# Snoworday/instance-segmentation-attention

Measured on NVIDIA B200. Metric: images/sec (pred.py inference, train step at 1/2/4/8 B200) vs host-CPU ref, higher is better.
Workload: dtype f32 (hot path fp32-accurate: bf16x3 tensor-core products, fp32 accumulation; cuDNN backbone convolutions at PyTorch's default TF32)

## Files before the change

### instance-segmentation-attention_b200/csrc/proj_gemm.cu

```cuda
#include "isa_common.cuh"
#include "isa_tcgen05.cuh"

namespace {

constexpr int kBM = 256;
constexpr int kBNMax = 256;
constexpr int kBK = 32;
constexpr int kStages = 3;
constexpr int kProducerThreads = 512;
constexpr int kThreadsTotal = kProducerThreads;
constexpr int kTileA = kBM * kBK * 2;
constexpr int kTileB = kBNMax * kBK * 2;
constexpr int kStageBytes = 2 * kTileA + 2 * kTileB;
constexpr int kGroupStride = (kBK / 8) * 128;
constexpr int kMaxSeg = 4;

struct Seg {
  const float* ptr;
  long long ld;
  long long shift;
  int cols;
  int v0;
  int pos_div, pos_mod, pos_step;
  int ones;
};

struct Operand {
  Seg seg[kMaxSeg];
  int nseg;
  int mn_major;
  int extent;
};

struct GemmParams {
  Operand a, b;
  long long K;
  long long k_per_split;
  float* out;
  long long ldc;
  long long out_rows;
  int out_cols;
  int bn;
  const unsigned char* b_packed;
  int n_iter_total;
};

struct Chunk {
  const float* p;
  long long step;
  int off;
  int k0;
  int tail;
  int seg;
};

__device__ __forceinline__ void plan_chunk(const Operand& op, long long mn_base, int groups, long long k_lo, int q, Chunk& c) {
  c.p = nullptr; c.step = 0; c.off = 0; c.k0 = 0; c.tail = 8; c.seg = -1;
  if (op.mn_major) {
    const int k8 = q & 7, mgl = (q >> 3) & 3, rest = q >> 5, kg = rest & 3, mg = (rest >> 2) * 4 + mgl;
    if (mg >= groups) { c.off = -1; return; }
    c.off = mg * kGroupStride + kg * 128 + k8 * 16;
    c.k0 = (int)k_lo + kg * 8 + k8;
    const int mn0 = (int)mn_base + mg * 8;
    if (mn0 >= op.extent) return;
    int si = 0;
#pragma unroll
    for (int j = 1; j < kMaxSeg; ++j)
      if (j < op.nseg && mn0 >= op.seg[j].v0) si = j;
    const Seg& sg = op.seg[si];
    const int col = mn0 - sg.v0;
    if (col >= sg.cols) return;
    c.tail = sg.cols - col < 8 ? sg.cols - col : 8;
    c.seg = (sg.ones || sg.pos_step != 0) ? si : -1;
    c.step = (long long)kBK * sg.ld;
    c.p = sg.ones ? reinterpret_cast<const float*>(&op)  : sg.ptr + ((long long)c.k0 + sg.shift) * sg.ld + col;
  } else {
    const int r8 = q & 7, kc = (q >> 3) & 3, rg = q >> 5;
    if (rg >= groups) { c.off = -1; return; }
    c.off = rg * kGroupStride + kc * 128 + r8 * 16;
    c.k0 = (int)k_lo + kc * 8;
    const long long mn = mn_base + rg * 8 + r8;
    if (mn >= op.extent) return;
    c.step = kBK;
    c.p = op.seg[0].ptr + mn * op.seg[0].ld + c.k0;
  }
}

__device__ __forceinline__ void load_chunk(const Operand& op, const Chunk& c, int it, int k_hi, float (&v)[8]) {
#pragma unroll
  for (int i = 0; i < 8; ++i) v[i] = 0.f;
  if (c.p == nullptr) return;
  const int k = c.k0 + it * kBK;
  if (k >= k_hi) return;
  const float* p = c.p + (long long)it * c.step;
  if (op.mn_major) {
    if (c.seg >= 0) {
      const Seg& sg = op.seg[c.seg];
      if (sg.ones) {
#pragma unroll
        for (int i = 0; i < 8; ++i) v[i] = i < c.tail ? 1.f : 0.f;
        return;
      }
      const int pos = (int)(((unsigned)k / (unsigned)sg.pos_div) % (unsigned)sg.pos_mod) + sg.pos_step;
      if (pos < 0 || pos >= sg.pos_mod) return;
    }
    if (c.tail == 8) {
      const float4 a = __ldg(reinterpret_cast<const float4*>(p));
      const float4 b = __ldg(reinterpret_cast<const float4*>(p + 4));
      v[0] = a.x; v[1] = a.y; v[2] = a.z; v[3] = a.w; v[4] = b.x; v[5] = b.y; v[6] = b.z; v[7] = b.w;
    } else {
#pragma unroll
      for (int i = 0; i < 8; ++i)
        if (i < c.tail) v[i] = __ldg(p + i);
    }
  } else {
    if (k + 8 <= k_hi) {
      const float4 a = __ldg(reinterpret_cast<const float4*>(p));
      const float4 b = __ldg(reinterpret_cast<const float4*>(p + 4));
      v[0] = a.x; v[1] = a.y; v[2] = a.z; v[3] = a.w; v[4] = b.x; v[5] = b.y; v[6] = b.z; v[7] = b.w;
    } else {
#pragma unroll
      for (int i = 0; i < 8; ++i)
        if (k + i < k_hi) v[i] = __ldg(p + i);
    }
  }
}

__device__ __forceinline__ void store_split8(unsigned char* hi_tile, unsigned char* lo_tile, int off, const float (&v)[8]) {
  uint4 h, l;
  split2(v[0], v[1], h.x, l.x);
  split2(v[2], v[3], h.y, l.y);
  split2(v[4], v[5], h.z, l.z);
  split2(v[6], v[7], h.w, l.w);
  *reinterpret_cast<uint4*>(hi_tile + off) = h;
  *reinterpret_cast<uint4*>(lo_tile + off) = l;
}

__global__ void __launch_bounds__(kProducerThreads) pack_operand_kernel(const __grid_constant__ Operand op, int bn, int k_total, unsigned char* __restrict__ dst) {
  const int it = blockIdx.x, nt = blockIdx.y;
  const int n0 = nt * bn;
  int width = op.extent - n0;
  width = width > bn ? bn : ((width + 15) & ~15);
  unsigned char* hi = dst + ((size_t)nt * gridDim.x + it) * 2 * (size_t)bn * (kBK * 2);
  unsigned char* lo = hi + (size_t)bn * (kBK * 2);
#pragma unroll 1
  for (int i = 0; i < kBNMax * (kBK / 8) / kProducerThreads; ++i) {
    Chunk c;
    plan_chunk(op, n0, width / 8, 0, threadIdx.x + i * kProducerThreads, c);
    if (c.off < 0) continue;
    float v[8];
    load_chunk(op, c, it, k_total, v);
    store_split8(hi, lo, c.off, v);
  }
}

template <bool PACKED_B>
__global__ void __launch_bounds__(kThreadsTotal, 1) proj_gemm_kernel(const __grid_constant__ GemmParams p) {
  extern __shared__ __align__(16) unsigned char smem_raw_g[];
  unsigned char* sm = smem_raw_g + ((128u - (smem_u32(smem_raw_g) & 127u)) & 127u);
  __shared__ uint64_t s_full[kStages], s_empty[kStages], s_done;
  __shared__ uint32_t s_tmem;
  const int tid = threadIdx.x;
  const int warp = __shfl_sync(0xffffffffu, tid >> 5, 0);
  const long long m0 = (long long)blockIdx.y * kBM;
  const int n0 = blockIdx.x * p.bn;
  const long long k_lo = (long long)blockIdx.z * p.k_per_split;
  const int k_hi = (int)((k_lo + p.k_per_split < p.K) ? k_lo + p.k_per_split : p.K);
  const int n_iter = (int)((k_hi - k_lo + kBK - 1) / kBK);
  int bn = p.b.extent - n0;
  bn = bn > p.bn ? p.bn : ((bn + 15) & ~15);
  const int n_acc = (p.a.extent - m0 > 128) ? 2 : 1;

  if (tid == 0) {
    for (int s = 0; s < kStages; ++s) { mbar_init(&s_full[s], kProducerThreads / 32 + (PACKED_B ? 1 : 0)); mbar_init(&s_empty[s], 1); }
    mbar_init(&s_done, 1);
    fence_barrier_init();
  }
  if (warp == 0) tmem_alloc(&s_tmem, 512);
  tc_fence_before();
  __syncthreads();
  tc_fence_after();
  const uint32_t tmem = s_tmem;

  {
    const uint32_t el = elect_one();
    const uint32_t idesc = make_idesc(128, bn) | ((uint32_t)(p.a.mn_major ? 1 : 0) << 15) | ((uint32_t)(p.b.mn_major ? 1 : 0) << 16);
    constexpr int NA = kBM * (kBK / 8) / kProducerThreads;
    constexpr int NB = PACKED_B ? 1 : kBNMax * (kBK / 8) / kProducerThreads;
    Chunk ca[NA], cb[NB];
    float va[NA][8], vb[NB][8], na[NA][8], nb_[NB][8];
#pragma unroll
    for (int i = 0; i < NA; ++i) {
      plan_chunk(p.a, m0, n_acc * 16, k_lo, tid + i * kProducerThreads, ca[i]);
      if (ca[i].off >= 0) load_chunk(p.a, ca[i], 0, k_hi, va[i]);
    }
    if (!PACKED_B) {
#pragma unroll
      for (int i = 0; i < NB; ++i) {
        plan_chunk(p.b, n0, bn / 8, k_lo, tid + i * kProducerThreads, cb[i]);
        if (cb[i].off >= 0) load_chunk(p.b, cb[i], 0, k_hi, vb[i]);
      }
    }
    const size_t pk_tile = (size_t)p.bn * (kBK * 2);
    const int lane_p = tid & 31;
    auto k_block = [&](int it, float (&cur_a)[NA][8], float (&cur_b)[NB][8], float (&nxt_a)[NA][8], float (&nxt_b)[NB][8]) {
      const int s = it % kStages;
      const uint32_t ph = (uint32_t)(it / kStages) & 1u;
      if (it + 1 < n_iter) {
#pragma unroll
        for (int i = 0; i < NA; ++i)
          if (ca[i].off >= 0) load_chunk(p.a, ca[i], it + 1, k_hi, nxt_a[i]);
        if (!PACKED_B) {
#pragma unroll
          for (int i = 0; i < NB; ++i)
            if (cb[i].off >= 0) load_chunk(p.b, cb[i], it + 1, k_hi, nxt_b[i]);
        }
      }
      if (lane_p == 0) mbar_wait(&s_empty[s], ph ^ 1u);
      __syncwarp();
      unsigned char* st = sm + s * kStageBytes;
      if (PACKED_B && tid == 0) {
        const unsigned char* src = p.b_packed + ((size_t)blockIdx.x * p.n_iter_total + (size_t)(k_lo / kBK) + it) * 2 * pk_tile;
        const uint32_t bytes = (uint32_t)bn * (kBK * 2);
        mbar_arrive_expect_tx(&s_full[s], 2 * bytes);
        tma_bulk_g2s(st + 2 * kTileA, src, bytes, &s_full[s]);
        tma_bulk_g2s(st + 2 * kTileA + kTileB, src + pk_tile, bytes, &s_full[s]);
      }
#pragma unroll
      for (int i = 0; i < NA; ++i)
        if (ca[i].off >= 0) store_split8(st, st + kTileA, ca[i].off, cur_a[i]);
      if (!PACKED_B) {
#pragma unroll
        for (int i = 0; i < NB; ++i)
          if (cb[i].off >= 0) store_split8(st + 2 * kTileA, st + 2 * kTileA + kTileB, cb[i].off, cur_b[i]);
      }
      fence_proxy_async();
      __syncwarp();
      if (lane_p == 0) mbar_arrive(&s_full[s]);
      if (warp == 0) {
        mbar_wait(&s_full[s], ph);
        tc_fence_after();
        const uint32_t base = smem_u32(st);
        const uint64_t b_hi = make_desc(base + 2 * kTileA, 128, kGroupStride), b_lo = make_desc(base + 2 * kTileA + kTileB, 128, kGroupStride);
        for (int acc = 0; acc < n_acc; ++acc) {
          const uint32_t a_off = (uint32_t)acc * (16 * kGroupStride);
          const uint64_t a_hi = make_desc(base + a_off, 128, kGroupStride), a_lo = make_desc(base + kTileA + a_off, 128, kGroupStride);
          const uint32_t d = tmem + (uint32_t)acc * 256u;
#pragma unroll
          for (int kk = 0; kk < kBK / 16; ++kk) {
            const uint64_t ko = (uint64_t)((kk * 256) >> 4);
            umma_bf16_e(el, d, a_hi + ko, b_hi + ko, idesc, (it > 0 || kk > 0) ? 1u : 0u);
            umma_bf16_e(el, d, a_hi + ko, b_lo + ko, idesc, 1u);
            umma_bf16_e(el, d, a_lo + ko, b_hi + ko, idesc, 1u);
          }
        }
        umma_commit_e(el, &s_empty[s]);
        if (it + 1 == n_iter) umma_commit_e(el, &s_done);
      }
    };
    for (int it = 0; it < n_iter; it += 2) {
      k_block(it, va, vb, na, nb_);
      if (it + 1 < n_iter) k_block(it + 1, na, nb_, va, vb);
    }
    if (warp < 4 * n_acc) {
      mbar_wait(&s_done, 0);
      tc_fence_after();
      const int lane = tid & 31;
      const int acc = warp >> 2, quarter = warp & 3;
      const uint32_t t_row = tmem + ((uint32_t)(quarter * 32) << 16) + (uint32_t)acc * 256u;
      float* stg = reinterpret_cast<float*>(sm) + warp * (32 * 36);
      const long long row_base = m0 + acc * 128 + quarter * 32;
      float* obase = p.out + ((long long)blockIdx.z * p.out_rows + row_base) * p.ldc + n0;
      for (int c0 = 0; c0 < bn; c0 += 32) {
        uint32_t d[32];
        if (bn - c0 >= 32) {
          tmem_ld32_issue(t_row + c0, d);
          tmem_ld32_wait(d);
        } else {
          uint32_t e[16];
          tmem_ld16_issue(t_row + c0, e);
          tmem_ld16_wait(e);
#pragma unroll
          for (int i = 0; i < 16; ++i) { d[i] = e[i]; d[i + 16] = 0u; }
        }
#pragma unroll
        for (int i = 0; i < 32; i += 4) *reinterpret_cast<uint4*>(stg + lane * 36 + i) = make_uint4(d[i], d[i + 1], d[i + 2], d[i + 3]);
        __syncwarp();
        int lim = p.out_cols - (n0 + c0);
        if (lim > bn - c0) lim = bn - c0;
        const int col = (lane & 7) * 4;
#pragma unroll
        for (int j = 0; j < 8; ++j) {
          const int r = j * 4 + (lane >> 3);
          const uint4 v = *reinterpret_cast<const uint4*>(stg + r * 36 + col);
          if (row_base + r < p.out_rows) {
            float* o = obase + (long long)r * p.ldc + c0 + col;
            if (col + 4 <= lim) *reinterpret_cast<uint4*>(o) = v;
            else {
              if (col + 0 < lim) o[0] = __uint_as_float(v.x);
              if (col + 1 < lim) o[1] = __uint_as_float(v.y);
              if (col + 2 < lim) o[2] = __uint_as_float(v.z);
              if (col + 3 < lim) o[3] = __uint_as_float(v.w);
            }
          }
        }
        __syncwarp();
      }
      tc_fence_before();
    }
  }
  __syncthreads();
  if (warp == 0) {
    tc_fence_after();
    tmem_dealloc(tmem, 512);
  }
}

__global__ void __launch_bounds__(256) renet_wgrad_reduce_kernel(const float* __restrict__ part, int splits, long long rows_pad, long long ldc,
                                                                 int n, int cin, int cb0, int cb1, int cone, float* __restrict__ dw_ih,
                                                                 float* __restrict__ dw_hh, float* __restrict__ db_ih, float* __restrict__ db_hh) {
  const int n_ih = 6 * n * cin, n_hh = 2 * 3 * n * n, n_b = 6 * n;
  const int total = n_ih + n_hh + 2 * n_b;
  for (int i = blockIdx.x * blockDim.x + threadIdx.x; i < total; i += gridDim.x * blockDim.x) {
    int r, c;
    float* dst;
    if (i < n_ih) { r = i / cin; c = i % cin; dst = dw_ih + i; }
    else if (i < n_ih + n_hh) {
      const int j = i - n_ih;
      const int d = j / (3 * n * n), g = (j / n) % (3 * n), u = j % n;
      r = g < 2 * n ? d * 3 * n + g : 6 * n + d * n + (g - 2 * n);
      c = (d == 0 ? cb0 : cb1) + u;
      dst = dw_hh + j;
    } else if (i < n_ih + n_hh + n_b) { r = i - n_ih - n_hh; c = cone; dst = db_ih + r; }
    else {
      const int j = i - n_ih - n_hh - n_b;
      const int d = j / (3 * n), g = j % (3 * n);
      r = g < 2 * n ? d * 3 * n + g : 6 * n + d * n + (g - 2 * n);
      c = cone;
      dst = db_hh + j;
    }
    float acc = 0.f;
    for (int s = 0; s < splits; ++s) acc += part[((long long)s * rows_pad + r) * ldc + c];
    *dst = acc;
  }
}

Seg plain_seg(const float* ptr, long long ld, int cols, int v0) {
  Seg s;
  s.ptr = ptr; s.ld = ld; s.shift = 0; s.cols = cols; s.v0 = v0; s.pos_div = 1; s.pos_mod = 1; s.pos_step = 0; s.ones = 0;
  return s;
}

int pick_bn(int extent) {
  const int tiles = (extent + kBNMax - 1) / kBNMax;
  int bn = (extent + tiles - 1) / tiles;
  return (bn + 15) & ~15;
}

int pick_bn_fwd(int extent) { return pick_bn(extent); }

int launch_gemm(const GemmParams& p, long long M, int splits, cudaStream_t stream) {
  static thread_local bool attr_set[16] = {false};
  IsaDeviceInfo di;
  int rc = isa_device_info(&di);
  if (rc) return rc;
  const size_t smem = (size_t)kStages * kStageBytes + 128;
  if (di.device >= 0 && di.device < 16 && !attr_set[di.device]) {
    ISA_CUDA(cudaFuncSetAttribute(proj_gemm_kernel<false>, cudaFuncAttributeMaxDynamicSharedMemorySize, (int)smem));
    ISA_CUDA(cudaFuncSetAttribute(proj_gemm_kernel<true>, cudaFuncAttributeMaxDynamicSharedMemorySize, (int)smem));
    attr_set[di.device] = true;
  }
  dim3 grid((unsigned)((p.b.extent + p.bn - 1) / p.bn), (unsigned)((M + kBM - 1) / kBM), (unsigned)splits);
  if (p.b_packed) proj_gemm_kernel<true><<<grid, kThreadsTotal, smem, stream>>>(p);
  else proj_gemm_kernel<false><<<grid, kThreadsTotal, smem, stream>>>(p);
  ISA_CUDA(cudaGetLastError());
  return ISA_OK;
}

int pack_b(GemmParams& p, void* workspace, size_t workspace_bytes, const char* who, cudaStream_t stream) {
  const int n_tiles = (p.b.extent + p.bn - 1) / p.bn;
  const int k_blocks = (int)((p.K + kBK - 1) / kBK);
  const size_t need = (size_t)n_tiles * k_blocks * 2 * p.bn * (kBK * 2);
  if (workspace == nullptr || workspace_bytes < need) {
    isa_set_error("%s: workspace %zu < %zu", who, workspace_bytes, need);
    return ISA_ERR_WORKSPACE;
  }
  pack_operand_kernel<<<dim3(k_blocks, n_tiles), kProducerThreads, 0, stream>>>(p.b, p.bn, (int)p.K, reinterpret_cast<unsigned char*>(workspace));
  ISA_CUDA(cudaGetLastError());
  p.b_packed = reinterpret_cast<const unsigned char*>(workspace);
  p.n_iter_total = k_blocks;
  return ISA_OK;
}

size_t pack_bytes(int extent, int K) {
  const int bn = pick_bn_fwd(extent);
  const int n_tiles = (extent + bn - 1) / bn;
  const int k_blocks = (K + kBK - 1) / kBK;
  return (size_t)n_tiles * k_blocks * 2 * bn * (kBK * 2);
}

bool aligned16(const void* p) { return (reinterpret_cast<uintptr_t>(p) & 15u) == 0; }

}

extern "C" {

size_t isa_renet_proj_workspace_bytes(int cin, int n_out) {
  if (cin <= 0 || n_out <= 0) return 0;
  const size_t a = pack_bytes(n_out, cin);
  const size_t b = pack_bytes((cin + 7) & ~7, n_out);
  return a > b ? a : b;
}

int isa_renet_proj_fwd(const float* x, const float* w, long long tokens, int cin, int n_out, float* gx, void* workspace,
                       size_t workspace_bytes, cudaStream_t stream) {
  ISA_CHECK_ARG(x && w && gx, "renet_proj_fwd: null pointer");
  ISA_CHECK_ARG(tokens > 0 && cin > 0 && n_out > 0 && cin % 4 == 0 && n_out % 4 == 0,
                "renet_proj_fwd: tokens=%lld cin=%d n_out=%d (widths must be positive multiples of 4)", tokens, cin, n_out);
  ISA_CHECK_ARG(aligned16(x) && aligned16(w) && aligned16(gx) && aligned16(workspace), "renet_proj_fwd: pointers must be 16-byte aligned");
  ISA_CHECK_ARG(tokens < 0x7fffffff, "renet_proj_fwd: too many tokens");
  GemmParams p;
  p.a.nseg = 1; p.a.mn_major = 0; p.a.extent = (int)tokens;
  p.a.seg[0] = plain_seg(x, cin, cin, 0);
  p.b.nseg = 1; p.b.mn_major = 0; p.b.extent = n_out;
  p.b.seg[0] = plain_seg(w, cin, cin, 0);
  p.K = cin; p.k_per_split = ((cin + kBK - 1) / kBK) * kBK;
  p.out = gx; p.ldc = n_out; p.out_rows = tokens; p.out_cols = n_out;
  p.bn = pick_bn(n_out);
  int rc = pack_b(p, workspace, workspace_bytes, "renet_proj_fwd", stream);
  if (rc) return rc;
  return launch_gemm(p, tokens, 1, stream);
}

int isa_renet_proj_dx(const float* dg, const float* w, long long tokens, int n_out, int cin, float* dx, void* workspace,
                      size_t workspace_bytes, cudaStream_t stream) {
  ISA_CHECK_ARG(dg && w && dx, "renet_proj_dx: null pointer");
  ISA_CHECK_ARG(tokens > 0 && tokens < 0x7fffffff && cin > 0 && n_out > 0 && cin % 4 == 0 && n_out % 4 == 0,
                "renet_proj_dx: tokens=%lld cin=%d n_out=%d (widths must be positive multiples of 4)", tokens, cin, n_out);
  ISA_CHECK_ARG(aligned16(dg) && aligned16(w) && aligned16(dx) && aligned16(workspace), "renet_proj_dx: pointers must be 16-byte aligned");
  GemmParams p;
  p.a.nseg = 1; p.a.mn_major = 0; p.a.extent = (int)tokens;
  p.a.seg[0] = plain_seg(dg, n_out, n_out, 0);
  p.b.nseg = 1; p.b.mn_major = 1; p.b.extent = (cin + 7) & ~7;
  p.b.seg[0] = plain_seg(w, cin, cin, 0);
  p.K = n_out; p.k_per_split = ((n_out + kBK - 1) / kBK) * kBK;
  p.out = dx; p.ldc = cin; p.out_rows = tokens; p.out_cols = cin;
  p.bn = pick_bn(p.b.extent);
  int rc = pack_b(p, workspace, workspace_bytes, "renet_proj_dx", stream);
  if (rc) return rc;
  return launch_gemm(p, tokens, 1, stream);
}

static void wgrad_geometry(int n, int cin, long long tokens, int num_sms, int* cb0, int* cb1, int* cone, int* nb, long long* rows_pad,
                           int* splits, long long* k_per) {
  const int nv = (n + 7) & ~7, cv = (cin + 7) & ~7;
  *cb0 = cv; *cb1 = cv + nv; *cone = cv + 2 * nv; *nb = cv + 2 * nv + 8;
  const long long m_tiles = (8LL * n + kBM - 1) / kBM;
  *rows_pad = m_tiles * kBM;
  const int n_tiles = (*nb + pick_bn(*nb) - 1) / pick_bn(*nb);
  long long tiles = m_tiles * n_tiles;
  int s = (int)((long long)num_sms / tiles);
  const long long max_s = (tokens + 4 * kBK - 1) / (4 * kBK);
  if (s > max_s) s = (int)max_s;
  if (s < 1) s = 1;
  long long kp = (tokens + s - 1) / s;
  kp = (kp + kBK - 1) / kBK * kBK;
  *splits = (int)((tokens + kp - 1) / kp);
  *k_per = kp;
}

size_t isa_renet_proj_wgrad_workspace_bytes(long long tokens, int cin, int n) {
  if (tokens <= 0 || cin <= 0 || n <= 0) return 0;
  IsaDeviceInfo di;
  if (isa_device_info(&di) != ISA_OK) { di.num_sms = 148; }
  int cb0, cb1, cone, nb, splits;
  long long rows_pad, kper;
  wgrad_geometry(n, cin, tokens, di.num_sms, &cb0, &cb1, &cone, &nb, &rows_pad, &splits, &kper);
  return (size_t)splits * rows_pad * nb * sizeof(float);
}

int isa_renet_proj_wgrad(const float* dgx, const float* dghn, const float* x, const float* out, long long tokens, int cin, int n,
                         long long step, int pos_div, int pos_mod, float* dw_ih, float* dw_hh, float* db_ih, float* db_hh,
                         void* workspace, size_t workspace_bytes, cudaStream_t stream) {
  ISA_CHECK_ARG(dgx && dghn && x && out && dw_ih && dw_hh && db_ih && db_hh && workspace, "renet_proj_wgrad: null pointer");
  ISA_CHECK_ARG(tokens > 0 && tokens < 0x7fffffff && cin > 0 && n > 0 && cin % 4 == 0 && n % 4 == 0,
                "renet_proj_wgrad: tokens=%lld cin=%d n=%d (widths must be positive multiples of 4)", tokens, cin, n);
  ISA_CHECK_ARG(pos_div > 0 && pos_mod > 0 && step > 0, "renet_proj_wgrad: step / pos_div / pos_mod must be positive");
  ISA_CHECK_ARG(aligned16(dgx) && aligned16(dghn) && aligned16(x) && aligned16(out), "renet_proj_wgrad: pointers must be 16-byte aligned");
  IsaDeviceInfo di;
  int rc = isa_device_info(&di);
  if (rc) return rc;
  int cb0, cb1, cone, nb, splits;
  long long rows_pad, kper;
  wgrad_geometry(n, cin, tokens, di.num_sms, &cb0, &cb1, &cone, &nb, &rows_pad, &splits, &kper);
  const size_t need = (size_t)splits * rows_pad * nb * sizeof(float);
  if (workspace_bytes < need) {
    isa_set_error("renet_proj_wgrad: workspace %zu < %zu", workspace_bytes, need);
    return ISA_ERR_WORKSPACE;
  }
  GemmParams p;
  p.a.nseg = 2; p.a.mn_major = 1; p.a.extent = 8 * n;
  p.a.seg[0] = plain_seg(dgx, 6LL * n, 6 * n, 0);
  p.a.seg[1] = plain_seg(dghn, 2LL * n, 2 * n, 6 * n);
  ISA_CHECK_ARG((6 * n) % 8 == 0, "renet_proj_wgrad: 6 n must be a multiple of 8 (n = %d)", n);
  p.b.nseg = 4; p.b.mn_major = 1; p.b.extent = nb;
  p.b.seg[0] = plain_seg(x, cin, cin, 0);
  p.b.seg[1] = plain_seg(out, 2LL * n, n, cb0);
  p.b.seg[1].shift = -step; p.b.seg[1].pos_div = pos_div; p.b.seg[1].pos_mod = pos_mod; p.b.seg[1].pos_step = -1;
  p.b.seg[2] = plain_seg(out + n, 2LL * n, n, cb1);
  p.b.seg[2].shift = step; p.b.seg[2].pos_div = pos_div; p.b.seg[2].pos_mod = pos_mod; p.b.seg[2].pos_step = 1;
  p.b.seg[3] = plain_seg(nullptr, 0, 1, cone);
  p.b.seg[3].ones = 1;
  p.K = tokens; p.k_per_split = kper;
  p.out = reinterpret_cast<float*>(workspace); p.ldc = nb; p.out_rows = rows_pad; p.out_cols = nb;
  p.bn = pick_bn(nb);
  p.b_packed = nullptr; p.n_iter_total = 0;
  rc = launch_gemm(p, 8LL * n, splits, stream);
  if (rc) return rc;
  const int total = 6 * n * cin + 6 * n * n + 12 * n;
  int blocks = (total + 255) / 256;
  if (blocks > di.num_sms * 8) blocks = di.num_sms * 8;
  renet_wgrad_reduce_kernel<<<blocks, 256, 0, stream>>>(reinterpret_cast<const float*>(workspace), splits, rows_pad, nb, n, cin, cb0, cb1, cone,
                                                        dw_ih, dw_hh, db_ih, db_hh);
  ISA_CUDA(cudaGetLastError());
  return ISA_OK;
}

}
```

Measured before the change: 1546.

## Split renet wgrad into per-problem tiled kernel and simplify projection GEMM

Replaces the generic segmented-operand GEMM used for the weight gradient with a dedicated wgrad kernel. It schedules a list of per-problem output tiles with their own split-K counts, so it only computes the blocks that are actually needed instead of a padded concatenated matrix. The forward and dx GEMMs drop the segment machinery and the template branch, and always use a packed B operand. This reduces wasted MMA work and per-chunk segment and position branching, but adds a tile-table limit, more complex planning code, and a new reduce kernel.

```diff
diff --git a/instance-segmentation-attention_b200/csrc/proj_gemm.cu b/instance-segmentation-attention_b200/csrc/proj_gemm.cu
--- a/instance-segmentation-attention_b200/csrc/proj_gemm.cu
+++ b/instance-segmentation-attention_b200/csrc/proj_gemm.cu
@@ -13,36 +13,28 @@
 constexpr int kTileB = kBNMax * kBK * 2;
 constexpr int kStageBytes = 2 * kTileA + 2 * kTileB;
 constexpr int kGroupStride = (kBK / 8) * 128;
-constexpr int kMaxSeg = 4;
-
-struct Seg {
+constexpr size_t kSmemBytes = (size_t)kStages * kStageBytes + 128;
+
+struct Operand {
   const float* ptr;
   long long ld;
-  long long shift;
   int cols;
-  int v0;
-  int pos_div, pos_mod, pos_step;
-  int ones;
-};
-
-struct Operand {
-  Seg seg[kMaxSeg];
-  int nseg;
   int mn_major;
   int extent;
 };
 
 struct GemmParams {
-  Operand a, b;
-  long long K;
-  long long k_per_split;
+  Operand a;
+  int K;
+  int n_iter;
   float* out;
   long long ldc;
   long long out_rows;
   int out_cols;
+  int b_extent;
+  int b_mn_major;
   int bn;
   const unsigned char* b_packed;
-  int n_iter_total;
 };
 
 struct Chunk {
@@ -51,38 +43,35 @@
   int off;
   int k0;
   int tail;
-  int seg;
 };
 
-__device__ __forceinline__ void plan_chunk(const Operand& op, long long mn_base, int groups, long long k_lo, int q, Chunk& c) {
-  c.p = nullptr; c.step = 0; c.off = 0; c.k0 = 0; c.tail = 8; c.seg = -1;
+__device__ __forceinline__ int mn_chunk(int q, int groups, int& krow, int& mg) {
+  const int k8 = q & 7, mgl = (q >> 3) & 3, rest = q >> 5, kg = rest & 3;
+  mg = (rest >> 2) * 4 + mgl;
+  krow = kg * 8 + k8;
+  return mg >= groups ? -1 : mg * kGroupStride + kg * 128 + k8 * 16;
+}
+
+__device__ __forceinline__ void plan_chunk(const Operand& op, int mn_base, int groups, int q, Chunk& c) {
+  c.p = nullptr; c.step = 0; c.off = 0; c.k0 = 0; c.tail = 8;
   if (op.mn_major) {
-    const int k8 = q & 7, mgl = (q >> 3) & 3, rest = q >> 5, kg = rest & 3, mg = (rest >> 2) * 4 + mgl;
-    if (mg >= groups) { c.off = -1; return; }
-    c.off = mg * kGroupStride + kg * 128 + k8 * 16;
-    c.k0 = (int)k_lo + kg * 8 + k8;
-    const int mn0 = (int)mn_base + mg * 8;
-    if (mn0 >= op.extent) return;
-    int si = 0;
-#pragma unroll
-    for (int j = 1; j < kMaxSeg; ++j)
-      if (j < op.nseg && mn0 >= op.seg[j].v0) si = j;
-    const Seg& sg = op.seg[si];
-    const int col = mn0 - sg.v0;
-    if (col >= sg.cols) return;
-    c.tail = sg.cols - col < 8 ? sg.cols - col : 8;
-    c.seg = (sg.ones || sg.pos_step != 0) ? si : -1;
-    c.step = (long long)kBK * sg.ld;
-    c.p = sg.ones ? reinterpret_cast<const float*>(&op)  : sg.ptr + ((long long)c.k0 + sg.shift) * sg.ld + col;
+    int mg;
+    c.off = mn_chunk(q, groups, c.k0, mg);
+    if (c.off < 0) return;
+    const int mn0 = mn_base + mg * 8;
+    if (mn0 >= op.cols) return;
+    c.tail = op.cols - mn0 < 8 ? op.cols - mn0 : 8;
+    c.step = (long long)kBK * op.ld;
+    c.p = op.ptr + (long long)c.k0 * op.ld + mn0;
   } else {
     const int r8 = q & 7, kc = (q >> 3) & 3, rg = q >> 5;
     if (rg >= groups) { c.off = -1; return; }
     c.off = rg * kGroupStride + kc * 128 + r8 * 16;
-    c.k0 = (int)k_lo + kc * 8;
-    const long long mn = mn_base + rg * 8 + r8;
+    c.k0 = kc * 8;
+    const long long mn = (long long)mn_base + rg * 8 + r8;
     if (mn >= op.extent) return;
     c.step = kBK;
-    c.p = op.seg[0].ptr + mn * op.seg[0].ld + c.k0;
+    c.p = op.ptr + mn * op.ld + c.k0;
   }
 }
 
@@ -93,36 +82,15 @@
   const int k = c.k0 + it * kBK;
   if (k >= k_hi) return;
   const float* p = c.p + (long long)it * c.step;
-  if (op.mn_major) {
-    if (c.seg >= 0) {
-      const Seg& sg = op.seg[c.seg];
-      if (sg.ones) {
-#pragma unroll
-        for (int i = 0; i < 8; ++i) v[i] = i < c.tail ? 1.f : 0.f;
-        return;
-      }
-      const int pos = (int)(((unsigned)k / (unsigned)sg.pos_div) % (unsigned)sg.pos_mod) + sg.pos_step;
-      if (pos < 0 || pos >= sg.pos_mod) return;
-    }
-    if (c.tail == 8) {
-      const float4 a = __ldg(reinterpret_cast<const float4*>(p));
-      const float4 b = __ldg(reinterpret_cast<const float4*>(p + 4));
-      v[0] = a.x; v[1] = a.y; v[2] = a.z; v[3] = a.w; v[4] = b.x; v[5] = b.y; v[6] = b.z; v[7] = b.w;
-    } else {
-#pragma unroll
-      for (int i = 0; i < 8; ++i)
-        if (i < c.tail) v[i] = __ldg(p + i);
-    }
+  const int lim = op.mn_major ? c.tail : k_hi - k;
+  if (lim >= 8) {
+    const float4 a = __ldg(reinterpret_cast<const float4*>(p));
+    const float4 b = __ldg(reinterpret_cast<const float4*>(p + 4));
+    v[0] = a.x; v[1] = a.y; v[2] = a.z; v[3] = a.w; v[4] = b.x; v[5] = b.y; v[6] = b.z; v[7] = b.w;
   } else {
-    if (k + 8 <= k_hi) {
-      const float4 a = __ldg(reinterpret_cast<const float4*>(p));
-      const float4 b = __ldg(reinterpret_cast<const float4*>(p + 4));
-      v[0] = a.x; v[1] = a.y; v[2] = a.z; v[3] = a.w; v[4] = b.x; v[5] = b.y; v[6] = b.z; v[7] = b.w;
-    } else {
-#pragma unroll
-      for (int i = 0; i < 8; ++i)
-        if (k + i < k_hi) v[i] = __ldg(p + i);
-    }
+#pragma unroll
+    for (int i = 0; i < 8; ++i)
+      if (i < lim) v[i] = __ldg(p + i);
   }
 }
 
@@ -134,6 +102,72 @@
   split2(v[6], v[7], h.w, l.w);
   *reinterpret_cast<uint4*>(hi_tile + off) = h;
   *reinterpret_cast<uint4*>(lo_tile + off) = l;
+}
+
+__device__ __forceinline__ void issue_stage(uint32_t el, uint32_t tmem, uint32_t cs, uint32_t base, int n_acc, uint32_t idesc, bool first) {
+  const uint64_t b_hi = make_desc(base + 2 * kTileA, 128, kGroupStride), b_lo = make_desc(base + 2 * kTileA + kTileB, 128, kGroupStride);
+  for (int acc = 0; acc < n_acc; ++acc) {
+    const uint32_t a_off = (uint32_t)acc * (16 * kGroupStride);
+    const uint64_t a_hi = make_desc(base + a_off, 128, kGroupStride), a_lo = make_desc(base + kTileA + a_off, 128, kGroupStride);
+    const uint32_t d = tmem + (uint32_t)acc * cs;
+#pragma unroll
+    for (int kk = 0; kk < kBK / 16; ++kk) {
+      const uint64_t ko = (uint64_t)((kk * 256) >> 4);
+      umma_bf16_e(el, d, a_hi + ko, b_hi + ko, idesc, (!first || kk > 0) ? 1u : 0u);
+      umma_bf16_e(el, d, a_hi + ko, b_lo + ko, idesc, 1u);
+      umma_bf16_e(el, d, a_lo + ko, b_hi + ko, idesc, 1u);
+    }
+  }
+}
+
+__device__ __forceinline__ void store_tile(uint32_t tmem, uint32_t cs, bool zero, unsigned char* sm, int warp, int bn, float* out,
+                                           long long ldc, long long rows, int cols) {
+  const int lane = threadIdx.x & 31;
+  const int acc = warp >> 2, quarter = warp & 3;
+  const uint32_t t_row = tmem + ((uint32_t)(quarter * 32) << 16) + (uint32_t)acc * cs;
+  float* stg = reinterpret_cast<float*>(sm) + warp * (32 * 36);
+  const int row_base = acc * 128 + quarter * 32;
+  float* obase = out + (long long)row_base * ldc;
+  for (int c0 = 0; c0 < bn; c0 += 32) {
+    uint32_t d[32];
+    if (bn - c0 >= 32) {
+      tmem_ld32_issue(t_row + c0, d);
+      tmem_ld32_wait(d);
+    } else {
+      uint32_t e[16];
+      tmem_ld16_issue(t_row + c0, e);
+      tmem_ld16_wait(e);
+#pragma unroll
+      for (int i = 0; i < 16; ++i) { d[i] = e[i]; d[i + 16] = 0u; }
+    }
+    if (zero) {
+#pragma unroll
+      for (int i = 0; i < 32; ++i) d[i] = 0u;
+    }
+#pragma unroll
+    for (int i = 0; i < 32; i += 4) *reinterpret_cast<uint4*>(stg + lane * 36 + i) = make_uint4(d[i], d[i + 1], d[i + 2], d[i + 3]);
+    __syncwarp();
+    int lim = cols - c0;
+    if (lim > bn - c0) lim = bn - c0;
+    const int col = (lane & 7) * 4;
+#pragma unroll
+    for (int j = 0; j < 8; ++j) {
+      const int r = j * 4 + (lane >> 3);
+      const uint4 v = *reinterpret_cast<const uint4*>(stg + r * 36 + col);
+      if (row_base + r < rows) {
+        float* o = obase + (long long)r * ldc + c0 + col;
+        if (col + 4 <= lim) *reinterpret_cast<uint4*>(o) = v;
+        else {
+          if (col + 0 < lim) o[0] = __uint_as_float(v.x);
+          if (col + 1 < lim) o[1] = __uint_as_float(v.y);
+          if (col + 2 < lim) o[2] = __uint_as_float(v.z);
+          if (col + 3 < lim) o[3] = __uint_as_float(v.w);
+        }
+      }
+    }
+    __syncwarp();
+  }
+  tc_fence_before();
 }
 
 __global__ void __launch_bounds__(kProducerThreads) pack_operand_kernel(const __grid_constant__ Operand op, int bn, int k_total, unsigned char* __restrict__ dst) {
@@ -146,7 +180,7 @@
 #pragma unroll 1
   for (int i = 0; i < kBNMax * (kBK / 8) / kProducerThreads; ++i) {
     Chunk c;
-    plan_chunk(op, n0, width / 8, 0, threadIdx.x + i * kProducerThreads, c);
+    plan_chunk(op, n0, width / 8, threadIdx.x + i * kProducerThreads, c);
     if (c.off < 0) continue;
     float v[8];
     load_chunk(op, c, it, k_total, v);
@@ -154,7 +188,6 @@
   }
 }
 
-template <bool PACKED_B>
 __global__ void __launch_bounds__(kThreadsTotal, 1) proj_gemm_kernel(const __grid_constant__ GemmParams p) {
   extern __shared__ __align__(16) unsigned char smem_raw_g[];
   unsigned char* sm = smem_raw_g + ((128u - (smem_u32(smem_raw_g) & 127u)) & 127u);
@@ -164,15 +197,13 @@
   const int warp = __shfl_sync(0xffffffffu, tid >> 5, 0);
   const long long m0 = (long long)blockIdx.y * kBM;
   const int n0 = blockIdx.x * p.bn;
-  const long long k_lo = (long long)blockIdx.z * p.k_per_split;
-  const int k_hi = (int)((k_lo + p.k_per_split < p.K) ? k_lo + p.k_per_split : p.K);
-  const int n_iter = (int)((k_hi - k_lo + kBK - 1) / kBK);
-  int bn = p.b.extent - n0;
+  const int n_iter = p.n_iter;
+  int bn = p.b_extent - n0;
   bn = bn > p.bn ? p.bn : ((bn + 15) & ~15);
   const int n_acc = (p.a.extent - m0 > 128) ? 2 : 1;
 
   if (tid == 0) {
-    for (int s = 0; s < kStages; ++s) { mbar_init(&s_full[s], kProducerThreads / 32 + (PACKED_B ? 1 : 0)); mbar_init(&s_empty[s], 1); }
+    for (int s = 0; s < kStages; ++s) { mbar_init(&s_full[s], kProducerThreads / 32 + 1); mbar_init(&s_empty[s], 1); }
     mbar_init(&s_done, 1);
     fence_barrier_init();
   }
@@ -184,43 +215,30 @@
 
   {
     const uint32_t el = elect_one();
-    const uint32_t idesc = make_idesc(128, bn) | ((uint32_t)(p.a.mn_major ? 1 : 0) << 15) | ((uint32_t)(p.b.mn_major ? 1 : 0) << 16);
+    const uint32_t idesc = make_idesc(128, bn) | ((uint32_t)p.b_mn_major << 16);
     constexpr int NA = kBM * (kBK / 8) / kProducerThreads;
-    constexpr int NB = PACKED_B ? 1 : kBNMax * (kBK / 8) / kProducerThreads;
-    Chunk ca[NA], cb[NB];
-    float va[NA][8], vb[NB][8], na[NA][8], nb_[NB][8];
+    Chunk ca[NA];
+    float va[NA][8], na[NA][8];
 #pragma unroll
     for (int i = 0; i < NA; ++i) {
-      plan_chunk(p.a, m0, n_acc * 16, k_lo, tid + i * kProducerThreads, ca[i]);
-      if (ca[i].off >= 0) load_chunk(p.a, ca[i], 0, k_hi, va[i]);
-    }
-    if (!PACKED_B) {
-#pragma unroll
-      for (int i = 0; i < NB; ++i) {
-        plan_chunk(p.b, n0, bn / 8, k_lo, tid + i * kProducerThreads, cb[i]);
-        if (cb[i].off >= 0) load_chunk(p.b, cb[i], 0, k_hi, vb[i]);
-      }
+      plan_chunk(p.a, (int)m0, n_acc * 16, tid + i * kProducerThreads, ca[i]);
+      if (ca[i].off >= 0) load_chunk(p.a, ca[i], 0, p.K, va[i]);
     }
     const size_t pk_tile = (size_t)p.bn * (kBK * 2);
     const int lane_p = tid & 31;
-    auto k_block = [&](int it, float (&cur_a)[NA][8], float (&cur_b)[NB][8], float (&nxt_a)[NA][8], float (&nxt_b)[NB][8]) {
+    auto k_block = [&](int it, float (&cur_a)[NA][8], float (&nxt_a)[NA][8]) {
       const int s = it % kStages;
       const uint32_t ph = (uint32_t)(it / kStages) & 1u;
       if (it + 1 < n_iter) {
 #pragma unroll
         for (int i = 0; i < NA; ++i)
-          if (ca[i].off >= 0) load_chunk(p.a, ca[i], it + 1, k_hi, nxt_a[i]);
-        if (!PACKED_B) {
-#pragma unroll
-          for (int i = 0; i < NB; ++i)
-            if (cb[i].off >= 0) load_chunk(p.b, cb[i], it + 1, k_hi, nxt_b[i]);
-        }
+          if (ca[i].off >= 0) load_chunk(p.a, ca[i], it + 1, p.K, nxt_a[i]);
       }
       if (lane_p == 0) mbar_wait(&s_empty[s], ph ^ 1u);
       __syncwarp();
       unsigned char* st = sm + s * kStageBytes;
-      if (PACKED_B && tid == 0) {
-        const unsigned char* src = p.b_packed + ((size_t)blockIdx.x * p.n_iter_total + (size_t)(k_lo / kBK) + it) * 2 * pk_tile;
+      if (tid == 0) {
+        const unsigned char* src = p.b_packed + ((size_t)blockIdx.x * n_iter + it) * 2 * pk_tile;
         const uint32_t bytes = (uint32_t)bn * (kBK * 2);
         mbar_arrive_expect_tx(&s_full[s], 2 * bytes);
         tma_bulk_g2s(st + 2 * kTileA, src, bytes, &s_full[s]);
@@ -229,31 +247,188 @@
 #pragma unroll
       for (int i = 0; i < NA; ++i)
         if (ca[i].off >= 0) store_split8(st, st + kTileA, ca[i].off, cur_a[i]);
-      if (!PACKED_B) {
-#pragma unroll
-        for (int i = 0; i < NB; ++i)
-          if (cb[i].off >= 0) store_split8(st + 2 * kTileA, st + 2 * kTileA + kTileB, cb[i].off, cur_b[i]);
-      }
       fence_proxy_async();
       __syncwarp();
       if (lane_p == 0) mbar_arrive(&s_full[s]);
       if (warp == 0) {
         mbar_wait(&s_full[s], ph);
         tc_fence_after();
-        const uint32_t base = smem_u32(st);
-        const uint64_t b_hi = make_desc(base + 2 * kTileA, 128, kGroupStride), b_lo = make_desc(base + 2 * kTileA + kTileB, 128, kGroupStride);
-        for (int acc = 0; acc < n_acc; ++acc) {
-          const uint32_t a_off = (uint32_t)acc * (16 * kGroupStride);
-          const uint64_t a_hi = make_desc(base + a_off, 128, kGroupStride), a_lo = make_desc(base + kTileA + a_off, 128, kGroupStride);
-          const uint32_t d = tmem + (uint32_t)acc * 256u;
-#pragma unroll
-          for (int kk = 0; kk < kBK / 16; ++kk) {
-            const uint64_t ko = (uint64_t)((kk * 256) >> 4);
-            umma_bf16_e(el, d, a_hi + ko, b_hi + ko, idesc, (it > 0 || kk > 0) ? 1u : 0u);
-            umma_bf16_e(el, d, a_hi + ko, b_lo + ko, idesc, 1u);
-            umma_bf16_e(el, d, a_lo + ko, b_hi + ko, idesc, 1u);
+        issue_stage(el, tmem, 256u, smem_u32(st), n_acc, idesc, it == 0);
+        umma_commit_e(el, &s_empty[s]);
+        if (it + 1 == n_iter) umma_commit_e(el, &s_done);
+      }
+    };
+    for (int it = 0; it < n_iter; it += 2) {
+      k_block(it, va, na);
+      if (it + 1 < n_iter) k_block(it + 1, na, va);
+    }
+    if (warp < 4 * n_acc) {
+      mbar_wait(&s_done, 0);
+      tc_fence_after();
+      store_tile(tmem, 256u, false, sm, warp, bn, p.out + m0 * p.ldc + n0, p.ldc, p.out_rows - m0, p.out_cols - n0);
+    }
+  }
+  __syncthreads();
+  if (warp == 0) {
+    tc_fence_after();
+    tmem_dealloc(tmem, 512);
+  }
+}
+
+struct WTile {
+  int prob;
+  int m0, n0, bn, n_acc;
+  int cta0, splits;
+  int k_per;
+  int sets;
+  long long part;
+};
+constexpr int kMaxWTiles = 64;
+
+struct WgradParams {
+  const float *dgx, *dghn, *x, *out;
+  float* part;
+  long long step;
+  int tokens, n, cin, cv, nv;
+  int pos_div, pos_mod, inc_r, inc_p;
+  int ntiles;
+  WTile t[kMaxWTiles];
+};
+
+struct WChunk {
+  const float* p;
+  int step;
+  int off;
+  int kind;
+  int tail;
+};
+
+__device__ __forceinline__ void plan_wchunk(const WgradParams& p, int prob, int side, int c, long long tok, WChunk& w) {
+  w.p = nullptr; w.step = 0; w.kind = 0; w.tail = 8;
+  const int n = p.n;
+  const float* base = nullptr;
+  int ld = 0, cols = 0;
+  if (side == 0) {
+    if (prob == 0) { base = p.dgx + c; ld = 6 * n; cols = 6 * n - c; }
+    else if (c < 2 * n) { base = p.dgx + (prob - 1) * 3 * n + c; ld = 6 * n; cols = 2 * n - c; }
+    else { base = p.dghn + (prob - 1) * n + (c - 2 * n); ld = 2 * n; cols = 3 * n - c; }
+  } else if (prob == 0) {
+    if (c == p.cv) { w.kind = 1; return; }
+    base = p.x + c; ld = p.cin; cols = p.cin - c;
+  } else {
+    if (c == p.nv) { w.kind = 1; return; }
+    base = p.out + (prob - 1) * n + c; ld = 2 * n; cols = n - c;
+    tok += prob == 1 ? -p.step : p.step;
+    w.kind = 2;
+  }
+  if (cols <= 0) { w.kind = 0; return; }
+  w.tail = cols < 8 ? cols : 8;
+  w.step = kBK * ld;
+  w.p = base + tok * ld;
+}
+
+__global__ void __launch_bounds__(kThreadsTotal, 1) wgrad_kernel(const __grid_constant__ WgradParams p) {
+  extern __shared__ __align__(16) unsigned char smem_raw_g[];
+  unsigned char* sm = smem_raw_g + ((128u - (smem_u32(smem_raw_g) & 127u)) & 127u);
+  __shared__ uint64_t s_full[kStages], s_empty[kStages], s_done;
+  __shared__ uint32_t s_tmem;
+  const int tid = threadIdx.x;
+  const int warp = __shfl_sync(0xffffffffu, tid >> 5, 0);
+  int ti = 0;
+  while (ti + 1 < p.ntiles && (int)blockIdx.x >= p.t[ti + 1].cta0) ++ti;
+  const WTile T = p.t[ti];
+  const int split = blockIdx.x - T.cta0;
+  const int k_lo = split * T.k_per;
+  const int k_hi = k_lo + T.k_per < p.tokens ? k_lo + T.k_per : p.tokens;
+  const int n_iter = (k_hi - k_lo + kBK - 1) / kBK;
+  const int per_set = (n_iter + T.sets - 1) / T.sets;
+  const uint32_t cs = T.bn <= 128 ? 128u : 256u;
+
+  if (tid == 0) {
+    for (int s = 0; s < kStages; ++s) { mbar_init(&s_full[s], kProducerThreads / 32); mbar_init(&s_empty[s], 1); }
+    mbar_init(&s_done, 1);
+    fence_barrier_init();
+  }
+  if (warp == 0) tmem_alloc(&s_tmem, 512);
+  tc_fence_before();
+  __syncthreads();
+  tc_fence_after();
+  const uint32_t tmem = s_tmem;
+
+  {
+    const uint32_t el = elect_one();
+    const uint32_t idesc = make_idesc(128, T.bn) | (1u << 15) | (1u << 16);
+    constexpr int NA = kBM * (kBK / 8) / kProducerThreads;
+    constexpr int NB = kBNMax * (kBK / 8) / kProducerThreads;
+    WChunk ca[NA], cb[NB];
+    int krow = 0;
+#pragma unroll
+    for (int i = 0; i < NA; ++i) {
+      int mg;
+      ca[i].off = mn_chunk(tid + i * kProducerThreads, T.n_acc * 16, krow, mg);
+      plan_wchunk(p, T.prob, 0, T.m0 + mg * 8, (long long)k_lo + krow, ca[i]);
+    }
+#pragma unroll
+    for (int i = 0; i < NB; ++i) {
+      int mg;
+      cb[i].off = mn_chunk(tid + i * kProducerThreads, T.bn / 8, krow, mg);
+      plan_wchunk(p, T.prob, 1, T.n0 + mg * 8, (long long)k_lo + krow, cb[i]);
+    }
+    int tok = k_lo + krow;
+    int pos_r = tok % p.pos_div, pos_q = (tok / p.pos_div) % p.pos_mod;
+    const int pos_edge = T.prob == 1 ? 0 : p.pos_mod - 1;
+    auto load = [&](float (&va)[NA][8], float (&vb)[NB][8]) {
+      const bool row_ok = tok < k_hi;
+      const bool hp_ok = row_ok && pos_q != pos_edge;
+      auto one = [&](WChunk& c, float (&v)[8]) {
+#pragma unroll
+        for (int i = 0; i < 8; ++i) v[i] = 0.f;
+        if (c.kind == 1) { v[0] = row_ok ? 1.f : 0.f; return; }
+        if (c.p != nullptr && (c.kind == 2 ? hp_ok : row_ok)) {
+          const float4 a = __ldg(reinterpret_cast<const float4*>(c.p));
+          v[0] = a.x; v[1] = a.y; v[2] = a.z; v[3] = a.w;
+          if (c.tail == 8) {
+            const float4 b = __ldg(reinterpret_cast<const float4*>(c.p + 4));
+            v[4] = b.x; v[5] = b.y; v[6] = b.z; v[7] = b.w;
           }
         }
+        c.p += c.step;
+      };
+#pragma unroll
+      for (int i = 0; i < NA; ++i)
+        if (ca[i].off >= 0) one(ca[i], va[i]);
+#pragma unroll
+      for (int i = 0; i < NB; ++i)
+        if (cb[i].off >= 0) one(cb[i], vb[i]);
+      tok += kBK;
+      pos_r += p.inc_r;
+      pos_q += p.inc_p;
+      if (pos_r >= p.pos_div) { pos_r -= p.pos_div; ++pos_q; }
+      if (pos_q >= p.pos_mod) pos_q -= p.pos_mod;
+    };
+    float va[NA][8], vb[NB][8], na[NA][8], nb_[NB][8];
+    load(va, vb);
+    const int lane_p = tid & 31;
+    auto k_block = [&](int it, float (&cur_a)[NA][8], float (&cur_b)[NB][8], float (&nxt_a)[NA][8], float (&nxt_b)[NB][8]) {
+      const int s = it % kStages;
+      const uint32_t ph = (uint32_t)(it / kStages) & 1u;
+      if (it + 1 < n_iter) load(nxt_a, nxt_b);
+      if (lane_p == 0) mbar_wait(&s_empty[s], ph ^ 1u);
+      __syncwarp();
+      unsigned char* st = sm + s * kStageBytes;
+#pragma unroll
+      for (int i = 0; i < NA; ++i)
+        if (ca[i].off >= 0) store_split8(st, st + kTileA, ca[i].off, cur_a[i]);
+#pragma unroll
+      for (int i = 0; i < NB; ++i)
+        if (cb[i].off >= 0) store_split8(st + 2 * kTileA, st + 2 * kTileA + kTileB, cb[i].off, cur_b[i]);
+      fence_proxy_async();
+      __syncwarp();
+      if (lane_p == 0) mbar_arrive(&s_full[s]);
+      if (warp == 0) {
+        mbar_wait(&s_full[s], ph);
+        tc_fence_after();
+        issue_stage(el, tmem + (uint32_t)((it / per_set) * T.n_acc) * cs, cs, smem_u32(st), T.n_acc, idesc, it % per_set == 0);
         umma_commit_e(el, &s_empty[s]);
         if (it + 1 == n_iter) umma_commit_e(el, &s_done);
       }
@@ -262,51 +437,13 @@
       k_block(it, va, vb, na, nb_);
       if (it + 1 < n_iter) k_block(it + 1, na, nb_, va, vb);
     }
-    if (warp < 4 * n_acc) {
+    if (warp < 4 * T.n_acc) {
       mbar_wait(&s_done, 0);
       tc_fence_after();
-      const int lane = tid & 31;
-      const int acc = warp >> 2, quarter = warp & 3;
-      const uint32_t t_row = tmem + ((uint32_t)(quarter * 32) << 16) + (uint32_t)acc * 256u;
-      float* stg = reinterpret_cast<float*>(sm) + warp * (32 * 36);
-      const long long row_base = m0 + acc * 128 + quarter * 32;
-      float* obase = p.out + ((long long)blockIdx.z * p.out_rows + row_base) * p.ldc + n0;
-      for (int c0 = 0; c0 < bn; c0 += 32) {
-        uint32_t d[32];
-        if (bn - c0 >= 32) {
-          tmem_ld32_issue(t_row + c0, d);
-          tmem_ld32_wait(d);
-        } else {
-          uint32_t e[16];
-          tmem_ld16_issue(t_row + c0, e);
-          tmem_ld16_wait(e);
-#pragma unroll
-          for (int i = 0; i < 16; ++i) { d[i] = e[i]; d[i + 16] = 0u; }
-        }
-#pragma unroll
-        for (int i = 0; i < 32; i += 4) *reinterpret_cast<uint4*>(stg + lane * 36 + i) = make_uint4(d[i], d[i + 1], d[i + 2], d[i + 3]);
-        __syncwarp();
-        int lim = p.out_cols - (n0 + c0);
-        if (lim > bn - c0) lim = bn - c0;
-        const int col = (lane & 7) * 4;
-#pragma unroll
-        for (int j = 0; j < 8; ++j) {
-          const int r = j * 4 + (lane >> 3);
-          const uint4 v = *reinterpret_cast<const uint4*>(stg + r * 36 + col);
-          if (row_base + r < p.out_rows) {
-            float* o = obase + (long long)r * p.ldc + c0 + col;
-            if (col + 4 <= lim) *reinterpret_cast<uint4*>(o) = v;
-            else {
-              if (col + 0 < lim) o[0] = __uint_as_float(v.x);
-              if (col + 1 < lim) o[1] = __uint_as_float(v.y);
-              if (col + 2 < lim) o[2] = __uint_as_float(v.z);
-              if (col + 3 < lim) o[3] = __uint_as_float(v.w);
-            }
-          }
-        }
-        __syncwarp();
-      }
-      tc_fence_before();
+      const int rows = T.n_acc * 128;
+      for (int j = 0; j < T.sets; ++j)
+        store_tile(tmem + (uint32_t)(j * T.n_acc) * cs, cs, j * per_set >= n_iter, sm, warp, T.bn,
+                   p.part + T.part + ((long long)split * T.sets + j) * rows * T.bn, T.bn, rows, T.bn);
     }
   }
   __syncthreads();
@@ -316,39 +453,32 @@
   }
 }
 
-__global__ void __launch_bounds__(256) renet_wgrad_reduce_kernel(const float* __restrict__ part, int splits, long long rows_pad, long long ldc,
-                                                                 int n, int cin, int cb0, int cb1, int cone, float* __restrict__ dw_ih,
-                                                                 float* __restrict__ dw_hh, float* __restrict__ db_ih, float* __restrict__ db_hh) {
+__global__ void __launch_bounds__(256) wgrad_reduce_kernel(const __grid_constant__ WgradParams p, float* __restrict__ dw_ih,
+                                                           float* __restrict__ dw_hh, float* __restrict__ db_ih, float* __restrict__ db_hh) {
+  const int n = p.n, cin = p.cin;
   const int n_ih = 6 * n * cin, n_hh = 2 * 3 * n * n, n_b = 6 * n;
   const int total = n_ih + n_hh + 2 * n_b;
   for (int i = blockIdx.x * blockDim.x + threadIdx.x; i < total; i += gridDim.x * blockDim.x) {
-    int r, c;
+    int prob, r, c;
     float* dst;
-    if (i < n_ih) { r = i / cin; c = i % cin; dst = dw_ih + i; }
+    if (i < n_ih) { prob = 0; r = i / cin; c = i % cin; dst = dw_ih + i; }
     else if (i < n_ih + n_hh) {
       const int j = i - n_ih;
-      const int d = j / (3 * n * n), g = (j / n) % (3 * n), u = j % n;
-      r = g < 2 * n ? d * 3 * n + g : 6 * n + d * n + (g - 2 * n);
-      c = (d == 0 ? cb0 : cb1) + u;
-      dst = dw_hh + j;
-    } else if (i < n_ih + n_hh + n_b) { r = i - n_ih - n_hh; c = cone; dst = db_ih + r; }
-    else {
-      const int j = i - n_ih - n_hh - n_b;
-      const int d = j / (3 * n), g = j % (3 * n);
-      r = g < 2 * n ? d * 3 * n + g : 6 * n + d * n + (g - 2 * n);
-      c = cone;
-      dst = db_hh + j;
-    }
+      prob = 1 + j / (3 * n * n); r = (j / n) % (3 * n); c = j % n; dst = dw_hh + j;
+    } else if (i < n_ih + n_hh + n_b) { const int j = i - n_ih - n_hh; prob = 0; r = j; c = p.cv; dst = db_ih + j; }
+    else { const int j = i - n_ih - n_hh - n_b; prob = 1 + j / (3 * n); r = j % (3 * n); c = p.nv; dst = db_hh + j; }
+    int ti = 0;
+    for (int k = 0; k < p.ntiles; ++k) {
+      const WTile& t = p.t[k];
+      if (t.prob == prob && r >= t.m0 && r < t.m0 + t.n_acc * 128 && c >= t.n0 && c < t.n0 + t.bn) ti = k;
+    }
+    const WTile& t = p.t[ti];
+    const long long tile = (long long)t.n_acc * 128 * t.bn;
+    const float* src = p.part + t.part + (long long)(r - t.m0) * t.bn + (c - t.n0);
     float acc = 0.f;
-    for (int s = 0; s < splits; ++s) acc += part[((long long)s * rows_pad + r) * ldc + c];
+    for (int s = 0; s < t.splits * t.sets; ++s) acc += src[s * tile];
     *dst = acc;
   }
-}
-
-Seg plain_seg(const float* ptr, long long ld, int cols, int v0) {
-  Seg s;
-  s.ptr = ptr; s.ld = ld; s.shift = 0; s.cols = cols; s.v0 = v0; s.pos_div = 1; s.pos_mod = 1; s.pos_step = 0; s.ones = 0;
-  return s;
 }
 
 int pick_bn(int extent) {
@@ -357,46 +487,101 @@
   return (bn + 15) & ~15;
 }
 
-int pick_bn_fwd(int extent) { return pick_bn(extent); }
-
-int launch_gemm(const GemmParams& p, long long M, int splits, cudaStream_t stream) {
-  static thread_local bool attr_set[16] = {false};
-  IsaDeviceInfo di;
-  int rc = isa_device_info(&di);
-  if (rc) return rc;
-  const size_t smem = (size_t)kStages * kStageBytes + 128;
-  if (di.device >= 0 && di.device < 16 && !attr_set[di.device]) {
-    ISA_CUDA(cudaFuncSetAttribute(proj_gemm_kernel<false>, cudaFuncAttributeMaxDynamicSharedMemorySize, (int)smem));
-    ISA_CUDA(cudaFuncSetAttribute(proj_gemm_kernel<true>, cudaFuncAttributeMaxDynamicSharedMemorySize, (int)smem));
-    attr_set[di.device] = true;
-  }
-  dim3 grid((unsigned)((p.b.extent + p.bn - 1) / p.bn), (unsigned)((M + kBM - 1) / kBM), (unsigned)splits);
-  if (p.b_packed) proj_gemm_kernel<true><<<grid, kThreadsTotal, smem, stream>>>(p);
-  else proj_gemm_kernel<false><<<grid, kThreadsTotal, smem, stream>>>(p);
-  ISA_CUDA(cudaGetLastError());
-  return ISA_OK;
-}
-
-int pack_b(GemmParams& p, void* workspace, size_t workspace_bytes, const char* who, cudaStream_t stream) {
-  const int n_tiles = (p.b.extent + p.bn - 1) / p.bn;
-  const int k_blocks = (int)((p.K + kBK - 1) / kBK);
-  const size_t need = (size_t)n_tiles * k_blocks * 2 * p.bn * (kBK * 2);
+long long wgrad_plan(int n, int cin, long long tokens, int num_sms, WgradParams& p) {
+  p.n = n; p.cin = cin; p.tokens = (int)tokens;
+  p.cv = (cin + 7) & ~7; p.nv = (n + 7) & ~7;
+  p.ntiles = 0;
+  double weight[kMaxWTiles], total = 0.0;
+  for (int prob = 0; prob < 3; ++prob) {
+    const int m_ext = prob == 0 ? 6 * n : 3 * n;
+    const int n_ext = (prob == 0 ? p.cv : p.nv) + 8;
+    const int bnp = pick_bn(n_ext);
+    for (int m0 = 0; m0 < m_ext; m0 += kBM)
+      for (int n0 = 0; n0 < n_ext; n0 += bnp) {
+        if (p.ntiles == kMaxWTiles) return -1;
+        WTile& t = p.t[p.ntiles];
+        t.prob = prob; t.m0 = m0; t.n0 = n0;
+        t.bn = n_ext - n0 > bnp ? bnp : ((n_ext - n0 + 15) & ~15);
+        t.n_acc = m_ext - m0 > 128 ? 2 : 1;
+        t.sets = 512 / (t.n_acc * (t.bn <= 128 ? 128 : 256));
+        const double rows = t.n_acc * 128.0;
+        weight[p.ntiles] = rows * t.bn > 48.0 * (rows + t.bn) ? rows * t.bn : 48.0 * (rows + t.bn);
+        total += weight[p.ntiles];
+        ++p.ntiles;
+      }
+  }
+  const long long max_s = (tokens + 4 * kBK - 1) / (4 * kBK);
+  const int budget = num_sms > p.ntiles ? num_sms : p.ntiles;
+  int used = 0;
+  for (int i = 0; i < p.ntiles; ++i) {
+    int s = (int)(budget * weight[i] / total);
+    if (s < 1) s = 1;
+    if (s > max_s) s = (int)max_s;
+    p.t[i].splits = s;
+    used += s;
+  }
+  for (; used < budget; ++used) {
+    int best = -1;
+    for (int i = 0; i < p.ntiles; ++i)
+      if (p.t[i].splits < max_s && (best < 0 || weight[i] / p.t[i].splits > weight[best] / p.t[best].splits)) best = i;
+    if (best < 0) break;
+    ++p.t[best].splits;
+  }
+  long long floats = 0;
+  int cta = 0;
+  for (int i = 0; i < p.ntiles; ++i) {
+    WTile& t = p.t[i];
+    long long kp = (tokens + t.splits - 1) / t.splits;
+    kp = (kp + kBK - 1) / kBK * kBK;
+    t.k_per = (int)kp;
+    t.splits = (int)((tokens + kp - 1) / kp);
+    t.cta0 = cta;
+    cta += t.splits;
+    t.part = floats;
+    floats += (long long)t.splits * t.sets * t.n_acc * 128 * t.bn;
+  }
+  return floats;
+}
+
+int pack_b(const Operand& b, int bn, int K, int k_blocks, void* workspace, size_t workspace_bytes, const char* who, cudaStream_t stream) {
+  const int n_tiles = (b.extent + bn - 1) / bn;
+  const size_t need = (size_t)n_tiles * k_blocks * 2 * bn * (kBK * 2);
   if (workspace == nullptr || workspace_bytes < need) {
     isa_set_error("%s: workspace %zu < %zu", who, workspace_bytes, need);
     return ISA_ERR_WORKSPACE;
   }
-  pack_operand_kernel<<<dim3(k_blocks, n_tiles), kProducerThreads, 0, stream>>>(p.b, p.bn, (int)p.K, reinterpret_cast<unsigned char*>(workspace));
+  pack_operand_kernel<<<dim3(k_blocks, n_tiles), kProducerThreads, 0, stream>>>(b, bn, K, reinterpret_cast<unsigned char*>(workspace));
   ISA_CUDA(cudaGetLastError());
+  return ISA_OK;
+}
+
+int launch_gemm(const Operand& a, const Operand& b, int K, float* out, long long ldc, int out_cols, void* workspace,
+                size_t workspace_bytes, const char* who, cudaStream_t stream) {
+  GemmParams p;
+  p.a = a; p.K = K; p.n_iter = (K + kBK - 1) / kBK;
+  p.out = out; p.ldc = ldc; p.out_rows = a.extent; p.out_cols = out_cols;
+  p.b_extent = b.extent; p.b_mn_major = b.mn_major; p.bn = pick_bn(b.extent);
   p.b_packed = reinterpret_cast<const unsigned char*>(workspace);
-  p.n_iter_total = k_blocks;
+  const int rc = pack_b(b, p.bn, K, p.n_iter, workspace, workspace_bytes, who, stream);
+  if (rc) return rc;
+  ISA_CUDA(cudaFuncSetAttribute(proj_gemm_kernel, cudaFuncAttributeMaxDynamicSharedMemorySize, (int)kSmemBytes));
+  dim3 grid((unsigned)((b.extent + p.bn - 1) / p.bn), (unsigned)((a.extent + kBM - 1) / kBM));
+  proj_gemm_kernel<<<grid, kThreadsTotal, kSmemBytes, stream>>>(p);
+  ISA_CUDA(cudaGetLastError());
   return ISA_OK;
 }
 
 size_t pack_bytes(int extent, int K) {
-  const int bn = pick_bn_fwd(extent);
+  const int bn = pick_bn(extent);
   const int n_tiles = (extent + bn - 1) / bn;
   const int k_blocks = (K + kBK - 1) / kBK;
   return (size_t)n_tiles * k_blocks * 2 * bn * (kBK * 2);
+}
+
+Operand operand(const float* ptr, long long ld, int cols, int mn_major, int extent) {
+  Operand o;
+  o.ptr = ptr; o.ld = ld; o.cols = cols; o.mn_major = mn_major; o.extent = extent;
+  return o;
 }
 
 bool aligned16(const void* p) { return (reinterpret_cast<uintptr_t>(p) & 15u) == 0; }
@@ -419,17 +604,8 @@
                 "renet_proj_fwd: tokens=%lld cin=%d n_out=%d (widths must be positive multiples of 4)", tokens, cin, n_out);
   ISA_CHECK_ARG(aligned16(x) && aligned16(w) && aligned16(gx) && aligned16(workspace), "renet_proj_fwd: pointers must be 16-byte aligned");
   ISA_CHECK_ARG(tokens < 0x7fffffff, "renet_proj_fwd: too many tokens");
-  GemmParams p;
-  p.a.nseg = 1; p.a.mn_major = 0; p.a.extent = (int)tokens;
-  p.a.seg[0] = plain_seg(x, cin, cin, 0);
-  p.b.nseg = 1; p.b.mn_major = 0; p.b.extent = n_out;
-  p.b.seg[0] = plain_seg(w, cin, cin, 0);
-  p.K = cin; p.k_per_split = ((cin + kBK - 1) / kBK) * kBK;
-  p.out = gx; p.ldc = n_out; p.out_rows = tokens; p.out_cols = n_out;
-  p.bn = pick_bn(n_out);
-  int rc = pack_b(p, workspace, workspace_bytes, "renet_proj_fwd", stream);
-  if (rc) return rc;
-  return launch_gemm(p, tokens, 1, stream);
+  return launch_gemm(operand(x, cin, cin, 0, (int)tokens), operand(w, cin, cin, 0, n_out), cin, gx, n_out, n_out, workspace,
+                     workspace_bytes, "renet_proj_fwd", stream);
 }
 
 int isa_renet_proj_dx(const float* dg, const float* w, long long tokens, int n_out, int cin, float* dx, void* workspace,
@@ -438,45 +614,17 @@
   ISA_CHECK_ARG(tokens > 0 && tokens < 0x7fffffff && cin > 0 && n_out > 0 && cin % 4 == 0 && n_out % 4 == 0,
                 "renet_proj_dx: tokens=%lld cin=%d n_out=%d (widths must be positive multiples of 4)", tokens, cin, n_out);
   ISA_CHECK_ARG(aligned16(dg) && aligned16(w) && aligned16(dx) && aligned16(workspace), "renet_proj_dx: pointers must be 16-byte aligned");
-  GemmParams p;
-  p.a.nseg = 1; p.a.mn_major = 0; p.a.extent = (int)tokens;
-  p.a.seg[0] = plain_seg(dg, n_out, n_out, 0);
-  p.b.nseg = 1; p.b.mn_major = 1; p.b.extent = (cin + 7) & ~7;
-  p.b.seg[0] = plain_seg(w, cin, cin, 0);
-  p.K = n_out; p.k_per_split = ((n_out + kBK - 1) / kBK) * kBK;
-  p.out = dx; p.ldc = cin; p.out_rows = tokens; p.out_cols = cin;
-  p.bn = pick_bn(p.b.extent);
-  int rc = pack_b(p, workspace, workspace_bytes, "renet_proj_dx", stream);
-  if (rc) return rc;
-  return launch_gemm(p, tokens, 1, stream);
-}
-
-static void wgrad_geometry(int n, int cin, long long tokens, int num_sms, int* cb0, int* cb1, int* cone, int* nb, long long* rows_pad,
-                           int* splits, long long* k_per) {
-  const int nv = (n + 7) & ~7, cv = (cin + 7) & ~7;
-  *cb0 = cv; *cb1 = cv + nv; *cone = cv + 2 * nv; *nb = cv + 2 * nv + 8;
-  const long long m_tiles = (8LL * n + kBM - 1) / kBM;
-  *rows_pad = m_tiles * kBM;
-  const int n_tiles = (*nb + pick_bn(*nb) - 1) / pick_bn(*nb);
-  long long tiles = m_tiles * n_tiles;
-  int s = (int)((long long)num_sms / tiles);
-  const long long max_s = (tokens + 4 * kBK - 1) / (4 * kBK);
-  if (s > max_s) s = (int)max_s;
-  if (s < 1) s = 1;
-  long long kp = (tokens + s - 1) / s;
-  kp = (kp + kBK - 1) / kBK * kBK;
-  *splits = (int)((tokens + kp - 1) / kp);
-  *k_per = kp;
+  return launch_gemm(operand(dg, n_out, n_out, 0, (int)tokens), operand(w, cin, cin, 1, (cin + 7) & ~7), n_out, dx, cin, cin, workspace,
+                     workspace_bytes, "renet_proj_dx", stream);
 }
 
 size_t isa_renet_proj_wgrad_workspace_bytes(long long tokens, int cin, int n) {
   if (tokens <= 0 || cin <= 0 || n <= 0) return 0;
   IsaDeviceInfo di;
   if (isa_device_info(&di) != ISA_OK) { di.num_sms = 148; }
-  int cb0, cb1, cone, nb, splits;
-  long long rows_pad, kper;
-  wgrad_geometry(n, cin, tokens, di.num_sms, &cb0, &cb1, &cone, &nb, &rows_pad, &splits, &kper);
-  return (size_t)splits * rows_pad * nb * sizeof(float);
+  WgradParams p;
+  const long long floats = wgrad_plan(n, cin, tokens, di.num_sms, p);
+  return floats < 0 ? 0 : (size_t)floats * sizeof(float);
 }
 
 int isa_renet_proj_wgrad(const float* dgx, const float* dghn, const float* x, const float* out, long long tokens, int cin, int n,
@@ -490,38 +638,27 @@
   IsaDeviceInfo di;
   int rc = isa_device_info(&di);
   if (rc) return rc;
-  int cb0, cb1, cone, nb, splits;
-  long long rows_pad, kper;
-  wgrad_geometry(n, cin, tokens, di.num_sms, &cb0, &cb1, &cone, &nb, &rows_pad, &splits, &kper);
-  const size_t need = (size_t)splits * rows_pad * nb * sizeof(float);
+  WgradParams p;
+  const long long floats = wgrad_plan(n, cin, tokens, di.num_sms, p);
+  ISA_CHECK_ARG(floats >= 0, "renet_proj_wgrad: cin=%d n=%d need more than %d output tiles", cin, n, kMaxWTiles);
+  const size_t need = (size_t)floats * sizeof(float);
   if (workspace_bytes < need) {
     isa_set_error("renet_proj_wgrad: workspace %zu < %zu", workspace_bytes, need);
     return ISA_ERR_WORKSPACE;
   }
-  GemmParams p;
-  p.a.nseg = 2; p.a.mn_major = 1; p.a.extent = 8 * n;
-  p.a.seg[0] = plain_seg(dgx, 6LL * n, 6 * n, 0);
-  p.a.seg[1] = plain_seg(dghn, 2LL * n, 2 * n, 6 * n);
-  ISA_CHECK_ARG((6 * n) % 8 == 0, "renet_proj_wgrad: 6 n must be a multiple of 8 (n = %d)", n);
-  p.b.nseg = 4; p.b.mn_major = 1; p.b.extent = nb;
-  p.b.seg[0] = plain_seg(x, cin, cin, 0);
-  p.b.seg[1] = plain_seg(out, 2LL * n, n, cb0);
-  p.b.seg[1].shift = -step; p.b.seg[1].pos_div = pos_div; p.b.seg[1].pos_mod = pos_mod; p.b.seg[1].pos_step = -1;
-  p.b.seg[2] = plain_seg(out + n, 2LL * n, n, cb1);
-  p.b.seg[2].shift = step; p.b.seg[2].pos_div = pos_div; p.b.seg[2].pos_mod = pos_mod; p.b.seg[2].pos_step = 1;
-  p.b.seg[3] = plain_seg(nullptr, 0, 1, cone);
-  p.b.seg[3].ones = 1;
-  p.K = tokens; p.k_per_split = kper;
-  p.out = reinterpret_cast<float*>(workspace); p.ldc = nb; p.out_rows = rows_pad; p.out_cols = nb;
-  p.bn = pick_bn(nb);
-  p.b_packed = nullptr; p.n_iter_total = 0;
-  rc = launch_gemm(p, 8LL * n, splits, stream);
-  if (rc) return rc;
+  p.dgx = dgx; p.dghn = dghn; p.x = x; p.out = out;
+  p.part = reinterpret_cast<float*>(workspace);
+  p.step = step;
+  p.pos_div = pos_div; p.pos_mod = pos_mod;
+  p.inc_r = kBK % pos_div; p.inc_p = (kBK / pos_div) % pos_mod;
+  const int ctas = p.t[p.ntiles - 1].cta0 + p.t[p.ntiles - 1].splits;
+  ISA_CUDA(cudaFuncSetAttribute(wgrad_kernel, cudaFuncAttributeMaxDynamicSharedMemorySize, (int)kSmemBytes));
+  wgrad_kernel<<<ctas, kThreadsTotal, kSmemBytes, stream>>>(p);
+  ISA_CUDA(cudaGetLastError());
   const int total = 6 * n * cin + 6 * n * n + 12 * n;
   int blocks = (total + 255) / 256;
   if (blocks > di.num_sms * 8) blocks = di.num_sms * 8;
-  renet_wgrad_reduce_kernel<<<blocks, 256, 0, stream>>>(reinterpret_cast<const float*>(workspace), splits, rows_pad, nb, n, cin, cb0, cb1, cone,
-                                                        dw_ih, dw_hh, db_ih, db_hh);
+  wgrad_reduce_kernel<<<blocks, 256, 0, stream>>>(p, dw_ih, dw_hh, db_ih, db_hh);
   ISA_CUDA(cudaGetLastError());
   return ISA_OK;
 }
```

New measurement: 1483, median of 6. 0.959x the previous value.
